# annikabrundyn/driving-dirty

Measured on AMD Instinct MI355X. Metric: 6-view scenes/sec fwd+bwd, roadmap model bs=32, higher is better.
Workload: dtype f32

## Files before the change

### driving-dirty_amd/csrc/linear.hip

```cpp
#include "dd_common.h"

namespace {

constexpr int KT = 64;
constexpr int WROW = KT + 4;
constexpr int NTD = 32;

template <int MT, bool GT>
__device__ __forceinline__ void linear_fwd_body(const float* __restrict__ X, const float* __restrict__ Wt, const float* __restrict__ bias,
                                                float* __restrict__ Y, float* __restrict__ part, int M, int N, int K, int tiles_per_split,
                                                unsigned char* __restrict__ Y8, float tau) {
  __shared__ __attribute__((aligned(16))) float wl[128 * WROW];
  __shared__ __attribute__((aligned(16))) float xl[MT * 32 * WROW];
  const int tid = threadIdx.x, lane = tid & 63;
  const int wave = __builtin_amdgcn_readfirstlane(tid >> 6);
  const int h = lane >> 5, r = lane & 31;
  const int n0 = blockIdx.x * 128;
  const int ntiles = (K + KT - 1) / KT;
  const int t0 = blockIdx.y * tiles_per_split;
  const int t1 = min(t0 + tiles_per_split, ntiles);
  const int lrow = tid >> 4, lch = tid & 15;

  f32x4 wreg[8], xreg[2 * MT];
  auto fetch = [&](int t) {
    const int kc = t * KT + lch * 4;
    const bool kok = kc < K;
#pragma unroll
    for (int p = 0; p < 8; ++p) {
      const int n = n0 + p * 16 + lrow;
      const f32x4 v = __builtin_nontemporal_load((const f32x4*)(Wt + (long)min(n, N - 1) * K + min(kc, K - 4)));
      wreg[p] = (kok && n < N) ? v : f32x4{0.f, 0.f, 0.f, 0.f};
    }
#pragma unroll
    for (int p = 0; p < 2 * MT; ++p) {
      const int m = p * 16 + lrow;
      const f32x4 v = *(const f32x4*)(X + (long)min(m, M - 1) * K + min(kc, K - 4));
      xreg[p] = (kok && m < M) ? v : f32x4{0.f, 0.f, 0.f, 0.f};
    }
  };

  f32x16 acc[MT];
#pragma unroll
  for (int mt = 0; mt < MT; ++mt)
#pragma unroll
    for (int i = 0; i < 16; ++i) acc[mt][i] = 0.f;

  if (t0 < t1) fetch(t0);
  for (int t = t0; t < t1; ++t) {
#pragma unroll
    for (int p = 0; p < 8; ++p) *(f32x4*)(wl + (p * 16 + lrow) * WROW + lch * 4) = wreg[p];
#pragma unroll
    for (int p = 0; p < 2 * MT; ++p) *(f32x4*)(xl + (p * 16 + lrow) * WROW + lch * 4) = xreg[p];
    __syncthreads();
    if (t + 1 < t1) fetch(t + 1);
#pragma unroll
    for (int s = 0; s < KT / 8; ++s) {
      const f32x4 b4 = *(const f32x4*)(wl + (wave * 32 + r) * WROW + 8 * s + 4 * h);
#pragma unroll
      for (int mt = 0; mt < MT; ++mt) {
        const f32x4 a4 = *(const f32x4*)(xl + (mt * 32 + r) * WROW + 8 * s + 4 * h);
        acc[mt] = DD_MFMA(a4.x, b4.x, acc[mt]);
        acc[mt] = DD_MFMA(a4.y, b4.y, acc[mt]);
        acc[mt] = DD_MFMA(a4.z, b4.z, acc[mt]);
        acc[mt] = DD_MFMA(a4.w, b4.w, acc[mt]);
      }
    }
    __syncthreads();
  }

  const int n = n0 + wave * 32 + r;
  const bool direct = gridDim.y == 1;
  const float bv = (direct && bias && n < N) ? bias[n] : 0.f;
  if constexpr (GT) {
    unsigned char* tile = (unsigned char*)wl;
#pragma unroll
    for (int mt = 0; mt < MT; ++mt)
#pragma unroll
      for (int i = 0; i < 16; ++i) {
        float sig, l1p;
        dd_sigmoid_softplus(acc[mt][i] + bv, sig, l1p);
        tile[(mt * 32 + dd_acc_row(i, lane)) * 128 + wave * 32 + r] = sig > tau;
      }
    __syncthreads();
    const bool vec = N % 16 == 0 && (uintptr_t)Y8 % 16 == 0;
    const int c = (tid & 7) * 16;
#pragma unroll
    for (int p = 0; p < MT; ++p) {
      const int m = p * 32 + (tid >> 3);
      if (m >= M || n0 + c >= N) continue;
      unsigned char* dst8 = Y8 + (long)m * N + n0 + c;
      if (vec) {
        *(u32x4*)dst8 = *(const u32x4*)(tile + m * 128 + c);
      } else {
        for (int j = 0; j < min(16, N - n0 - c); ++j) dst8[j] = tile[m * 128 + c + j];
      }
    }
  } else {
    float* dst = direct ? Y : part + (long)blockIdx.y * M * N;
#pragma unroll
    for (int mt = 0; mt < MT; ++mt)
#pragma unroll
      for (int i = 0; i < 16; ++i) {
        const int m = mt * 32 + dd_acc_row(i, lane);
        if (m < M && n < N) dst[(long)m * N + n] = acc[mt][i] + bv;
      }
  }
}

template <int MT>
__global__ __launch_bounds__(256) void linear_fwd_kernel(const float* __restrict__ X, const float* __restrict__ Wt,
                                                         const float* __restrict__ bias, float* __restrict__ Y,
                                                         float* __restrict__ part, int M, int N, int K,
                                                         int tiles_per_split) {
  linear_fwd_body<MT, false>(X, Wt, bias, Y, part, M, N, K, tiles_per_split, nullptr, 0.f);
}

template <int MT>
__global__ __launch_bounds__(256) void linear_sigmoid_gt_kernel(const float* __restrict__ X, const float* __restrict__ Wt,
                                                                const float* __restrict__ bias, unsigned char* __restrict__ Y8, float tau,
                                                                int M, int N, int K) {
  linear_fwd_body<MT, true>(X, Wt, bias, nullptr, nullptr, M, N, K, (K + KT - 1) / KT, Y8, tau);
}

__global__ __launch_bounds__(256) void splits_reduce_kernel(const float* __restrict__ part, const float* __restrict__ bias,
                                                            float* __restrict__ out, long elems, int nsplit, int ncols) {
  __shared__ float red[32][8];
  const int el = threadIdx.x & 7, g = threadIdx.x >> 3;
  const long e = (long)blockIdx.x * 8 + el;
  float s0 = 0.f, s1 = 0.f, s2 = 0.f, s3 = 0.f;
  if (e < elems) {
    int s = g;
    for (; s + 96 < nsplit; s += 128) {
      s0 += part[(long)(s + 0) * elems + e];
      s1 += part[(long)(s + 32) * elems + e];
      s2 += part[(long)(s + 64) * elems + e];
      s3 += part[(long)(s + 96) * elems + e];
    }
    for (; s < nsplit; s += 32) s0 += part[(long)s * elems + e];
  }
  red[g][el] = (s0 + s1) + (s2 + s3);
  __syncthreads();
  if (g != 0 || e >= elems) return;
  float v = 0.f;
#pragma unroll
  for (int i = 0; i < 32; ++i) v += red[i][el];
  if (bias) v += bias[e % ncols];
  out[e] = v;
}

__global__ __launch_bounds__(256) void splits_reduce_few_kernel(const float* __restrict__ part, const float* __restrict__ bias,
                                                                float* __restrict__ out, long elems, int nsplit, int ncols) {
  const long e = (long)blockIdx.x * blockDim.x + threadIdx.x;
  if (e >= elems) return;
  float v = 0.f;
  for (int s = 0; s < nsplit; ++s) v += part[(long)s * elems + e];
  if (bias) v += bias[e % ncols];
  out[e] = v;
}

static inline void launch_splits_reduce(const float* part, const float* bias, float* out, long elems, int nsplit, int ncols, hipStream_t st) {
  if (nsplit >= 16)
    hipLaunchKernelGGL(splits_reduce_kernel, dim3((unsigned)((elems + 7) / 8)), dim3(256), 0, st, part, bias, out, elems, nsplit, ncols);
  else
    hipLaunchKernelGGL(splits_reduce_few_kernel, dim3((unsigned)((elems + 255) / 256)), dim3(256), 0, st, part, bias, out, elems, nsplit, ncols);
}

template <int MT>
__global__ __launch_bounds__(256) void linear_dgrad_kernel(const float* __restrict__ dY, const float* __restrict__ Wt,
                                                           float* __restrict__ dX, float* __restrict__ part, int M,
                                                           int N, int K, int tiles_per_split) {
  __shared__ __attribute__((aligned(16))) float wl[NTD * 128];
  __shared__ __attribute__((aligned(16))) float gl[MT * 32 * (NTD + 4)];
  constexpr int GROW = NTD + 4;
  const int tid = threadIdx.x, lane = tid & 63;
  const int wave = __builtin_amdgcn_readfirstlane(tid >> 6);
  const int h = lane >> 5, r = lane & 31;
  const int c0 = blockIdx.x * 128;
  const int ntiles = (N + NTD - 1) / NTD;
  const int t0 = blockIdx.y * tiles_per_split;
  const int t1 = min(t0 + tiles_per_split, ntiles);
// ... 177 lines not shown
  }

#pragma unroll
  for (int a = 0; a < TN; ++a) {
#pragma unroll
    for (int i = 0; i < 16; ++i) {
      const int n = nbase + 32 * a + dd_acc_row(i, lane);
      if (n < N && kok) __builtin_nontemporal_store(f32x4{acc[a][0][i], acc[a][1][i], acc[a][2][i], acc[a][3][i]}, (f32x4*)(dW + (long)n * K + kcol));
    }
    if (db && kg == 0) {
      const float tot = bsum[a] + __shfl_xor(bsum[a], 32);
      const int n = nbase + 32 * a + r;
      if (h == 0 && n < N) db[n] = tot;
    }
  }
}

__global__ __launch_bounds__(256) void column_sum_kernel(const float* __restrict__ dY, float* __restrict__ db, int M, int N) {
  const int c = (blockIdx.x * 256 + threadIdx.x) * 4;
  if (c >= N) return;
  if (c + 4 <= N && N % 4 == 0) {
    f32x4 s = {0.f, 0.f, 0.f, 0.f};
    for (int m = 0; m < M; ++m) s += *(const f32x4*)(dY + (long)m * N + c);
    *(f32x4*)(db + c) = s;
  } else {
    for (int j = c; j < min(c + 4, N); ++j) {
      float s = 0.f;
      for (int m = 0; m < M; ++m) s += dY[(long)m * N + j];
      db[j] = s;
    }
  }
}

int pick_mt(int M) { return M <= 32 ? 1 : (M <= 64 ? 2 : 0); }
constexpr int MCHUNK = 64;

int pick_split(int blocks_other, int ntiles) {
  if (ntiles <= 8) return 1;
  int want = (2 * DD_NUM_CU + blocks_other - 1) / blocks_other;
  want = max(1, min(want, ntiles));
  return min(want, 512);
}

int check_linear(const char* who, int M, int N, int K) {
  DD_REQUIRE(M > 0 && N > 0 && K > 0, DD_ERR_BAD_ARG, "%s: non-positive size", who);
  DD_REQUIRE(K % 4 == 0 && N % 4 == 0, DD_ERR_UNSUPPORTED, "%s: N = %d and K = %d must be multiples of 4", who, N, K);
  return 0;
}

}

extern "C" {

int64_t dd_linear_workspace_bytes(int32_t m, int32_t n, int32_t k) {
  const int64_t mc = m < MCHUNK ? m : MCHUNK;
  const int64_t fwd = ((n + 127) / 128 >= 2 * DD_NUM_CU) ? 0 : (int64_t)512 * mc * n * 4;
  const int64_t dgr = ((k + 127) / 128 >= 2 * DD_NUM_CU) ? 0 : (int64_t)512 * mc * k * 4;
  return (fwd > dgr ? fwd : dgr) + 16;
}

int dd_linear_fwd(const float* x, const float* w, const float* bias, float* y, int32_t m, int32_t n, int32_t k,
                  void* workspace, int64_t workspace_bytes, void* stream) {
  if (int rc = check_linear("linear_fwd", m, n, k)) return rc;
  DD_REQUIRE(x && w && y, DD_ERR_BAD_ARG, "linear_fwd: NULL pointer");
  hipStream_t st = (hipStream_t)stream;
  const int nblk = (n + 127) / 128, ntiles = (k + KT - 1) / KT;
  const int split = pick_split(nblk, ntiles);
  const int tps = (ntiles + split - 1) / split;
  const int nsplit = (ntiles + tps - 1) / tps;
  float* part = (float*)workspace;
  if (nsplit > 1)
    DD_REQUIRE(workspace && workspace_bytes >= (int64_t)nsplit * min(m, MCHUNK) * n * 4, DD_ERR_WORKSPACE, "linear_fwd: workspace too small");
  const dim3 grid(nblk, nsplit);
  for (int m0 = 0; m0 < m; m0 += MCHUNK) {
// ... 38 lines not shown
}

int dd_linear_dgrad(const float* dy, const float* w, float* dx, int32_t m, int32_t n, int32_t k, void* workspace,
                    int64_t workspace_bytes, void* stream) {
  if (int rc = check_linear("linear_dgrad", m, n, k)) return rc;
  DD_REQUIRE(dy && w && dx, DD_ERR_BAD_ARG, "linear_dgrad: NULL pointer");
  hipStream_t st = (hipStream_t)stream;
  const int kblk = (k + 127) / 128, ntiles = (n + NTD - 1) / NTD;
  const int split = pick_split(kblk, ntiles);
  const int tps = (ntiles + split - 1) / split;
  const int nsplit = (ntiles + tps - 1) / tps;
  float* part = (float*)workspace;
  if (nsplit > 1)
    DD_REQUIRE(workspace && workspace_bytes >= (int64_t)nsplit * min(m, MCHUNK) * k * 4, DD_ERR_WORKSPACE, "linear_dgrad: workspace too small");
  const dim3 grid(kblk, nsplit);
  for (int m0 = 0; m0 < m; m0 += MCHUNK) {
    const int mc = min(MCHUNK, m - m0);
    const float* dyc = dy + (long)m0 * n;
    float* dxc = dx + (long)m0 * k;
    switch (pick_mt(mc)) {
      case 1: hipLaunchKernelGGL(linear_dgrad_kernel<1>, grid, dim3(256), 0, st, dyc, w, dxc, part, mc, n, k, tps); break;
      default: hipLaunchKernelGGL(linear_dgrad_kernel<2>, grid, dim3(256), 0, st, dyc, w, dxc, part, mc, n, k, tps); break;
    }
    DD_LAUNCH_CHECK("linear_dgrad");
    if (nsplit > 1) {
      const long elems = (long)mc * k;
      launch_splits_reduce(part, nullptr, dxc, elems, nsplit, k, st);
      DD_LAUNCH_CHECK("linear_dgrad reduce");
    }
  }
  return 0;
}

int dd_column_sum(const float* dy, float* dbias, int32_t m, int32_t n, void* stream) {
  DD_REQUIRE(dy && dbias && m > 0 && n > 0, DD_ERR_BAD_ARG, "column_sum: bad argument");
  DD_REQUIRE(n % 4 != 0 || ((uintptr_t)dy | (uintptr_t)dbias) % 16 == 0, DD_ERR_BAD_ARG, "column_sum: buffers must be 16-byte aligned");
  hipLaunchKernelGGL(column_sum_kernel, dim3((unsigned)((n + 1023) / 1024)), dim3(256), 0, (hipStream_t)stream, dy, dbias, m, n);
  DD_LAUNCH_CHECK("column_sum");
  return 0;
}

int dd_linear_wgrad(const float* dy, const float* x, float* dw, float* dbias, int32_t m, int32_t n, int32_t k,
                    void* stream) {
  DD_REQUIRE(m > 0 && n > 0 && k > 0, DD_ERR_BAD_ARG, "linear_wgrad: non-positive size");
  DD_REQUIRE(dy && x && dw, DD_ERR_BAD_ARG, "linear_wgrad: NULL pointer");
  hipStream_t st = (hipStream_t)stream;
  if (k >= 512 && k % 4 == 0 && ((uintptr_t)x % 16 == 0) && ((uintptr_t)dw % 16 == 0)) {
    const int gk = (k + 127) / 128;
    const long total = (long)((n + 31) / 32) * gk;
    hipLaunchKernelGGL((linear_wgrad_wide_kernel<1>), dim3((unsigned)((total + 3) / 4)), dim3(256), 0, st, dy, x, dw,
                       dbias, m, n, k, gk, total);
  } else if (n <= 256 || k > n) {
    const int gk = (k + 31) / 32;
    const long total = (long)((n + 127) / 128) * gk;
    hipLaunchKernelGGL((linear_wgrad_kernel<4, 1>), dim3((unsigned)((total + 3) / 4)), dim3(256), 0, st, dy, x, dw, dbias,
                       m, n, k, gk, total);
  } else {
    const int gk = (k + 63) / 64;
    const long total = (long)((n + 31) / 32) * gk;
    hipLaunchKernelGGL((linear_wgrad_kernel<1, 2>), dim3((unsigned)((total + 3) / 4)), dim3(256), 0, st, dy, x, dw, dbias,
                       m, n, k, gk, total);
  }
  DD_LAUNCH_CHECK("linear_wgrad");
  return 0;
}

// ... 2 lines not shown
```

### driving-dirty_amd/joint.py

```python
import torch
from torch import nn

from . import ops
from .autoencoder import BasicAE
from .lightning import LightningModule, hparam, pretrained_ae
from .roadmap import predict_map
from .spatial import RoadMapBoxesMergingCNN, SpatialMappingCNN, bb_coord_to_map, boxes_from_map, per_sample_inputs


class JointRoadMapBBox(LightningModule):
    def __init__(self, hparams):
        super().__init__()
        self.hparams = hparams
        self.ae = pretrained_ae(hparams)
        self.ae.decoder = None
        self.ae.encoder.c3_only = False
        self.fc1 = nn.Linear(self.ae.latent_dim, 800 * 800)
        self.space_map_cnn = SpatialMappingCNN()
        self.box_merge = RoadMapBoxesMergingCNN()
        precision = hparam(hparams, "precision", None)
        if precision is not None:
            if precision not in ("fp32", "fp32x3"):
                raise ValueError(f"precision must be 'fp32' or 'fp32x3', got {precision!r}")
            self.box_merge.precision = precision

    def forward(self, x, rm):
        x = tuple(t.contiguous() for t in x) if isinstance(x, (tuple, list)) else x.contiguous()
        wide4 = ops.wide_image(x)
        feat, pooled = self.ae.encoder.conv_feature_and_pooled(wide4)
        boxes = self.box_merge(feat, self.space_map_cnn(x), rm).squeeze(1)
        z = self.ae.encoder._tail(pooled, (None, None))
        logits = ops.linear(z, self.fc1.weight, self.fc1.bias).reshape(-1, 800, 800)
        return logits, boxes

    def predict_boxes(self, x, rm, threshold=0.5, min_pixels=1, max_boxes=256, fit="extent", pad_px=0.5, split_px=0, grow_iters=None):
        with torch.no_grad():
            return boxes_from_map(self(x, rm)[1], threshold, min_pixels, max_boxes, fit, pad_px, split_px, grow_iters)

    def predict_road_map(self, x, threshold=None):
        views = tuple(t.contiguous() for t in x) if isinstance(x, (tuple, list)) else x.contiguous()
        return predict_map(self, lambda: self.ae.encoder.forward_nhwc4(ops.wide_image(views)), threshold)

    def training_step(self, batch, batch_idx):
        sample, target, road_image = batch
        if per_sample_inputs(sample, road_image) and all(t.numel() % 4 == 0 for t in road_image) and len(road_image) <= ops.PTR_TABLE_MAX:
            dev = sample[0].device
            b = len(sample)
            target_bb = bb_coord_to_map(target, dev).to(dev).float()
            logits, boxes = self(tuple(sample), tuple(road_image))
            loss_rm, _ = ops.BceWithLogitsProbs.apply(logits.reshape(b, -1), tuple(road_image))
        else:
            sample = torch.stack(tuple(sample), dim=0) if isinstance(sample, (tuple, list)) else sample
            target_rm = torch.stack(tuple(road_image), dim=0).float()
            target_bb = bb_coord_to_map(target, sample.device).to(sample.device).float()
            logits, boxes = self(sample, target_rm.unsqueeze(1))
            b = target_rm.size(0)
            loss_rm = ops.BceWithLogits.apply(logits.reshape(b, -1), target_rm.reshape(b, -1))
        loss_bb = ops.BceProbs.apply(boxes.reshape(b, -1), target_bb.reshape(b, -1))
        loss = loss_rm + loss_bb
        return {"loss": loss, "log": {"train_loss": loss, "roadmap_loss": loss_rm, "bbox_loss": loss_bb}}

    def configure_optimizers(self):
        return torch.optim.Adam(self.parameters(), lr=self.hparams.learning_rate)
```

### driving-dirty_amd/ops.py

```python
import ctypes as C
import os

import torch

from . import _lib
from . import ddp as _ddp
from ._lib import ConvDesc, call, check, size

EPI_NONE, EPI_BIAS, EPI_BIAS_RELU, EPI_RELU_MASK = 0, 1, 2, 3
PACK_FWD, PACK_DGRAD_S1, PACK_DGRAD_S2 = 0, 1, 2

_stream, _p, _dev = _lib.stream, _lib.ptr, _lib.dev


def conv_out(n, stride):
    return (n + 2 - 3) // stride + 1


def conv_desc(batch, h, w, cin_real, stride, rows_per_task=0):
    return ConvDesc(batch, h, w, cin_real, 4 if cin_real == 3 else cin_real, 32, 3, stride, 1, rows_per_task)


def stitch6(views, mask_slot=-1, want_nhwc4=True, want_nchw=False, want_target=False):
    b, n, c, h, w = views.shape
# ... 844 lines not shown
                        g1 = conv_wino_dgrad_bits(g2, p2d, s1, d2)
                    else:
                        g1 = conv_dgrad_bits(g2, p2d, s1, d2)
                    dw1, db1 = conv_wgrad(x4, g1, d1)

            if C2_DGRAD_FIRST:
                c2_data_gradient()
                for hook in MFMA_PHASE2_HOOKS:
                    hook()
                c2_weight_gradient()
            else:
                c2_weight_gradient()
                for hook in MFMA_PHASE2_HOOKS:
                    hook()
                c2_data_gradient()
            del g2
            if reduced is not None:
                torch.cuda.current_stream().wait_event(reduced)
        return None, dw1, db1, dw2, db2, dw3, db3, None, None


def encoder_conv_stack(x4, c1, c2, c3, pool, rows_per_task=0):
    return EncoderConvStack.apply(x4, c1.weight, c1.bias, c2.weight, c2.bias, c3.weight, c3.bias, pool, rows_per_task)


def _linear_ws(m, n, k, device):
    nbytes = size("dd_linear_workspace_bytes", m, n, k)
    return torch.empty(nbytes, device=device, dtype=torch.uint8), nbytes


RANKB = {}


class Linear(torch.autograd.Function):

    @staticmethod
    def forward(ctx, x, weight, bias):
        m, k = x.shape
        n = weight.shape[0]
        _dev(x, "x")
        _dev(weight, "weight", (n, k))
        if bias is not None:
            _dev(bias, "bias", (n,))
        y = torch.empty((m, n), device=x.device, dtype=torch.float32)
        ws, nbytes = _linear_ws(m, n, k, x.device)
        call("dd_linear_fwd", x, weight, bias, y, m, n, k, ws, nbytes)
        ctx.save_for_backward(x, weight)
        ctx.has_bias = bias is not None
        return y

    @staticmethod
    def backward(ctx, dy):
        x, weight = ctx.saved_tensors
        m, k = x.shape
        n = weight.shape[0]
        dy = dy.contiguous()
        dx = dw = db = None
        if ctx.needs_input_grad[0]:
            dx = torch.empty_like(x)
            ws, nbytes = _linear_ws(m, n, k, x.device)
            call("dd_linear_dgrad", dy, weight, dx, m, n, k, ws, nbytes)
        sync = _ddp.FACTOR_SYNC.get(weight.data_ptr()) if _ddp.FACTOR_SYNC else None
        fused = RANKB.get(weight.data_ptr()) if RANKB else None
        taken = 0
        if sync is not None and ctx.needs_input_grad[1] and sync.linear_factors(weight, x, dy):
            if ctx.has_bias and ctx.needs_input_grad[2] and not (fused is not None and fused.factor_bias(weight, sync.world * m)):
                db = column_sum(dy)
        elif fused is not None and ctx.needs_input_grad[1] and (taken := fused.linear_factors(weight, x, dy)):
            if taken == 1 and ctx.has_bias and ctx.needs_input_grad[2]:
                db = column_sum(dy)
        elif ctx.needs_input_grad[1] or (ctx.has_bias and ctx.needs_input_grad[2]):
            dw = torch.empty_like(weight)
            db = torch.empty(n, device=x.device, dtype=torch.float32) if ctx.has_bias else None
            call("dd_linear_wgrad", dy, x, dw, db, m, n, k)
        return dx, dw, db


def linear(x, weight, bias):
    x = x.contiguous()
    if _ddp.FACTOR_SYNC and torch.is_grad_enabled() and weight.requires_grad:
        sync = _ddp.FACTOR_SYNC.get(weight.data_ptr())
        if sync is not None:
            sync.linear_input(weight, x)
    return Linear.apply(x, weight, bias)


def linear_sigmoid_gt(x, weight, bias, tau):
    x = x.detach().contiguous()
    m, k = x.shape
    n = weight.shape[0]
    _dev(x, "x")
    _dev(weight.detach(), "weight", (n, k))
    if bias is not None:
        _dev(bias.detach(), "bias", (n,))
    out = torch.empty((m, n), device=x.device, dtype=torch.uint8)
    call("dd_linear_sigmoid_gt", x, weight, bias, float(tau), out, m, n, k)
    return out.view(torch.bool)


def column_sum(dy):
    m, n = dy.shape
    _dev(dy, "dy")
    db = torch.empty(n, device=dy.device, dtype=torch.float32)
    call("dd_column_sum", dy, db, m, n)
    return db


# ... 168 lines not shown
        probs = torch.empty_like(logits)
        dz = torch.empty_like(logits) if ctx.needs_input_grad[0] else None
        if isinstance(target, (tuple, list)):
            b, per = len(target), _check_masks(target, n)
            if b > PTR_TABLE_MAX:
                target = _stack_masks(target, logits.shape)
        if isinstance(target, (tuple, list)):
            table = (C.c_void_p * b)(*[t.data_ptr() for t in target])
            call("dd_bce_logits_u8_ptrs", logits, table, b, per, loss, dz, probs, 1.0, _loss_ws(n, logits.device))
            ctx.save_for_backward(dz)
            ctx.mark_non_differentiable(probs)
            ctx.set_materialize_grads(False)
            return loss, probs
        if not target.is_cuda or not target.is_contiguous() or target.shape != logits.shape:
            raise _lib.HotpathError(f"bce: target must be a contiguous GPU tensor of shape {tuple(logits.shape)}")
        if target.dtype in (torch.bool, torch.uint8):
            call("dd_bce_logits_u8", logits, target, loss, dz, probs, n, 1.0, _loss_ws(n, logits.device))
        else:
            _dev(target, "target", logits.shape)
            call("dd_bce_logits", logits, target, loss, dz, probs, n, 1.0, _loss_ws(n, logits.device))
        ctx.save_for_backward(dz)
        ctx.mark_non_differentiable(probs)
        ctx.set_materialize_grads(False)
        return loss, probs

    @staticmethod
    def backward(ctx, g, _gp):
        (dz,) = ctx.saved_tensors
        if g is None:
            return None, None
        return _scaled_loss_grad(ctx, dz, g), None


class MseLoss(torch.autograd.Function):

    @staticmethod
    def forward(ctx, pred, target):
        _dev(pred, "pred")
        _dev(target, "target", pred.shape)
        n = pred.numel()
        loss = torch.empty((), device=pred.device, dtype=torch.float32)
        da = torch.empty_like(pred) if ctx.needs_input_grad[0] else None
        call("dd_mse", pred, target, loss, da, n, 1.0, _loss_ws(n, pred.device))
        ctx.save_for_backward(da)
        return loss

    @staticmethod
    def backward(ctx, g):
        (da,) = ctx.saved_tensors
        return _scaled_loss_grad(ctx, da, g), None


class BceProbs(torch.autograd.Function):

    @staticmethod
    def forward(ctx, probs, target):
        _dev(probs, "probs")
        _dev(target, "target", probs.shape)
        n = probs.numel()
        loss = torch.empty((), device=probs.device, dtype=torch.float32)
        dp = torch.empty_like(probs) if ctx.needs_input_grad[0] else None
        call("dd_bce_probs", probs, target, loss, dp, n, 1.0, _loss_ws(n, probs.device))
        ctx.save_for_backward(dp)
        return loss

    @staticmethod
# ... 150 lines not shown
```

### driving-dirty_amd/roadmap.py

```python
from argparse import ArgumentParser

import torch
from torch import nn
from torch.nn import functional as F

from . import ops
from .autoencoder import BasicAE
from .lightning import LightningModule, hparam, pretrained_ae


def predict_map(module, latent, threshold):
    if threshold is None:
        threshold = hparam(module.hparams, "rm_threshold", None)
    tau = 0.5 if threshold is None else float(threshold)
    modes = [(m, m.training) for m in module.modules()]
    module.eval()
    try:
        with torch.no_grad():
            y = ops.linear_sigmoid_gt(latent(), module.fc1.weight, module.fc1.bias, tau)
    finally:
        for m, was in modes:
            m.training = was
    return y.reshape(y.size(0), 800, 800)

# ... 22 lines not shown
        x = torch.stack(tuple(sample), dim=0) if isinstance(sample, (tuple, list)) else sample
        return ops.stitch6(x.contiguous(), want_nhwc4=False, want_nchw=True)[1]

    def _encode(self, sample, keeps=(None, None)):
        wide4 = ops.wide_image(sample, self.ae.encoder.precision)
        return self.ae.encoder.forward_nhwc4(wide4, keeps)

    def _logits(self, x, keeps=(None, None)):
        representations = self._encode(x, keeps)
        y = ops.linear(representations, self.fc1.weight, self.fc1.bias)
        return y.reshape(y.size(0), 800, 800)

    def forward(self, x, keeps=(None, None)):
        y = self._logits(x, keeps)
        return y, ops.sigmoid(y.detach())

    @property
    def rm_threshold(self):
        return hparam(self.hparams, "rm_threshold", None)

    @rm_threshold.setter
    def rm_threshold(self, value):
        self.hparams.rm_threshold = None if value is None else float(value)

    def predict_road_map(self, x, threshold=None):
        return predict_map(self, lambda: self._encode(x), threshold)

    def _run_step(self, batch, batch_idx, step_name, keeps=(None, None)):
        sample, target, road_image = batch
        logging = self.logger is not None and batch_idx % self.hparams.output_img_freq == 0
        per_sample = tuple(road_image)
        if (step_name == "train" and not logging and 0 < len(per_sample) <= ops.PTR_TABLE_MAX and
                all(t.is_cuda and t.is_contiguous() and t.dtype in (torch.bool, torch.uint8) and t.numel() % 4 == 0 for t in per_sample)):
            pred_rm = self._logits(sample, keeps)
            b = len(per_sample)
            loss, probs = ops.BceWithLogitsProbs.apply(pred_rm.reshape(b, -1), per_sample)
            return loss, None, pred_rm, probs.reshape(b, 800, 800)
        masks = torch.stack(per_sample, dim=0)
        pred_rm = self._logits(sample, keeps)
        target_rm = masks.float() if (logging or step_name != "train" or masks.dtype.is_floating_point) else masks
        batch_size = masks.size(0)
        loss_target = masks if masks.dtype in (torch.bool, torch.uint8) else target_rm
        loss, probs = ops.BceWithLogitsProbs.apply(pred_rm.reshape(batch_size, -1), loss_target.reshape(batch_size, -1).contiguous())
        pred_logit_rm = probs.reshape(batch_size, 800, 800)
        if logging:
            self._log_rm_images(self.wide_stitch_six_images(sample), target_rm, pred_logit_rm, step_name)
        return loss, target_rm, pred_rm, pred_logit_rm

    def _log_rm_images(self, x, target_rm, pred_rm, step_name, limit=1):
        exp = self.logger.experiment
        step = self.trainer.global_step if self.trainer is not None else 0
        exp.add_image(f"{step_name}_input_images", x[:limit][0], step)
        exp.add_image(f"{step_name}_target_roadmaps", target_rm[:limit], step)
        exp.add_image(f"{step_name}_pred_roadmaps", pred_rm[:limit].round(), step)

    def training_step(self, batch, batch_idx):
        if self.current_epoch >= self.hparams.unfreeze_epoch_no and self.frozen:
            self.frozen = False
            self.ae.unfreeze()
        train_loss, _, _, _ = self._run_step(batch, batch_idx, step_name="train")
        return {"loss": train_loss, "log": {"train_loss": train_loss}}

    def validation_step(self, batch, batch_idx):
        val_loss, target_rm, pred_rm, pred_logit_rm = self._run_step(batch, batch_idx, step_name="valid")
        val_ts = compute_ts_road_map(target_rm, pred_logit_rm)
        val_ts_rounded = ops.threat_score(target_rm.contiguous(), pred_logit_rm.contiguous(), round_b=True)
# ... 63 lines not shown
```

### include/dd_hotpath.h

```cpp
#ifndef DD_HOTPATH_H
#define DD_HOTPATH_H

#include <stdint.h>

#ifdef __cplusplus
extern "C" {
#endif

#define DD_ABI_VERSION 4

enum {
  DD_OK = 0,
  DD_ERR_UNSUPPORTED = 1,
  DD_ERR_BAD_ARG = 2,
  DD_ERR_LAUNCH = 3,
  DD_ERR_WORKSPACE = 4
};

enum {
  DD_EPI_NONE = 0,
  DD_EPI_BIAS = 1,
  DD_EPI_BIAS_RELU = 2,
  DD_EPI_RELU_MASK = 3
};
// ... 228 lines not shown
int dd_subsample_nhwc4_u8_ptrs(const unsigned char* const* mask_ptrs, float* dst, int32_t batch, int32_t h, int32_t w,
                               int32_t oh, int32_t ow, int32_t stride, int32_t offset, void* stream);
int dd_conv1ch_fwd(const float* taps4, const float* w, const float* bias, float* y, int32_t batch, int32_t sh, int32_t sw,
                   int32_t relu, void* stream);
int dd_conv1ch_fwd_phase3(const float* taps4, const float* w, const float* bias, float* y_phase, uint32_t* relu_bits, int32_t batch,
                          int32_t sh, int32_t sw, int32_t relu, void* stream);
int dd_conv1ch_wgrad_phase3(const float* taps4, const float* g_phase, float* dw, float* dbias, int32_t batch, int32_t sh, int32_t sw,
                            void* workspace, void* stream);
int dd_phase3_scatter(const float* src_phase, float* dst, int32_t batch, int32_t oh, int32_t ow, int32_t src_ph, int32_t src_pw, int32_t off,
                      int32_t dst_cstore, int32_t dst_coff, void* stream);
int dd_phase3_gather(const float* src, float* dst_phase, int32_t batch, int32_t oh, int32_t ow, int32_t dst_ph, int32_t dst_pw, int32_t off,
                     int32_t src_cstore, int32_t src_coff, void* stream);
int64_t dd_conv1ch_wgrad_workspace_bytes(void);
int dd_conv1ch_wgrad(const float* taps4, const float* g, float* dw, float* dbias, int32_t batch, int32_t sh, int32_t sw,
                     void* workspace, void* stream);
int dd_copy_channels(const float* src, float* dst, int64_t npix, int32_t channels, int32_t src_cstore, int32_t src_coff,
                     int32_t dst_cstore, int32_t dst_coff, void* stream);
int dd_copy_channels_window(const float* src, float* dst, int32_t batch, int32_t h, int32_t w, int32_t channels, int32_t src_mem_h,
                            int32_t src_mem_w, int32_t src_y0, int32_t src_x0, int32_t src_cstore, int32_t src_coff, int32_t dst_mem_h,
                            int32_t dst_mem_w, int32_t dst_y0, int32_t dst_x0, int32_t dst_cstore, int32_t dst_coff, void* stream);
int dd_add(const float* a, const float* b, float* out, int64_t n, void* stream);
int dd_bce_probs(const float* probs, const float* target, float* loss_out, float* dprobs, int64_t n, float grad_scale,
                 void* workspace, void* stream);

int64_t dd_linear_workspace_bytes(int32_t m, int32_t n, int32_t k);
int dd_linear_fwd(const float* x, const float* w, const float* bias, float* y, int32_t m, int32_t n, int32_t k,
                  void* workspace, int64_t workspace_bytes, void* stream);
int dd_linear_dgrad(const float* dy, const float* w, float* dx, int32_t m, int32_t n, int32_t k, void* workspace,
                    int64_t workspace_bytes, void* stream);
int dd_linear_sigmoid_gt(const float* x, const float* w, const float* bias, float tau, uint8_t* out, int32_t m, int32_t n, int32_t k,
                         void* stream);
int dd_linear_wgrad(const float* dy, const float* x, float* dw, float* dbias, int32_t m, int32_t n, int32_t k,
                    void* stream);
int dd_column_sum(const float* dy, float* dbias, int32_t m, int32_t n, void* stream);

int64_t dd_threat_score_workspace_bytes(void);
int dd_threat_score(const float* a, const float* b, float* out, int64_t n, int32_t round_b, void* workspace, void* stream);

enum { DD_TARGET_F32 = 0, DD_TARGET_U8 = 1 };
int dd_ts_hist(const float* prob, const void* target, int32_t target_dtype, int64_t n, int32_t bins, int64_t* hist, void* stream);

int64_t dd_label_components_workspace_bytes(int32_t batch, int32_t height, int32_t width);
int dd_label_components(const float* maps, float threshold, int32_t* labels, int32_t batch, int32_t height, int32_t width, void* stream);

int64_t dd_component_boxes_workspace_bytes(int32_t batch, int32_t height, int32_t width);
int dd_component_boxes(const float* maps, float threshold, int32_t min_pixels, int32_t max_boxes, float* boxes, int32_t* counts, int32_t batch,
                       int32_t height, int32_t width, void* workspace, int64_t workspace_bytes, void* stream);

int64_t dd_component_obb_workspace_bytes(int32_t batch, int32_t height, int32_t width, int32_t max_boxes);
int dd_component_obb(const float* maps, float threshold, int32_t min_pixels, int32_t max_boxes, float pad_px, float* boxes, int32_t* counts,
                     int64_t* moments, int32_t batch, int32_t height, int32_t width, void* workspace, int64_t workspace_bytes, void* stream);

int64_t dd_split_components_workspace_bytes(int32_t batch, int32_t height, int32_t width, int32_t split_px, int32_t grow_iters);
int dd_split_components(const float* maps, float threshold, int32_t split_px, int32_t grow_iters, int32_t* labels, int32_t batch, int32_t height,
                        int32_t width, void* workspace, int64_t workspace_bytes, void* stream);

int64_t dd_labelled_boxes_workspace_bytes(int32_t batch, int32_t height, int32_t width);
int dd_labelled_boxes(const int32_t* labels, int32_t min_pixels, int32_t max_boxes, float* boxes, int32_t* counts, int32_t batch, int32_t height,
                      int32_t width, void* workspace, int64_t workspace_bytes, void* stream);
int64_t dd_labelled_obb_workspace_bytes(int32_t batch, int32_t height, int32_t width, int32_t max_boxes);
int dd_labelled_obb(const int32_t* labels, int32_t min_pixels, int32_t max_boxes, float pad_px, float* boxes, int32_t* counts, int64_t* moments,
                    int32_t batch, int32_t height, int32_t width, void* workspace, int64_t workspace_bytes, void* stream);

int64_t dd_box_iou_ats_workspace_bytes(const int32_t* offsets1, const int32_t* offsets2, int32_t batch);
int dd_box_iou_ats(const void* boxes1, int32_t dtype1, const int32_t* offsets1, const void* boxes2, int32_t dtype2, const int32_t* offsets2,
                   float* iou, float* ats, int32_t batch, void* workspace, int64_t workspace_bytes, void* stream);
// ... 111 lines not shown
```

Before: 4358.

## Fuse roadmap head linear, sigmoid-BCE loss, logit gradient and dgrad in one kernel

Adds a fused training kernel for the final fc1 layer. In one pass it computes the 640k-wide logits, the BCE loss against the per-sample byte masks, dZ = (sigmoid - t)*scale, and partial input gradients dX. This avoids writing the logits to memory and reading them back in a separate BCE kernel, and replaces the separate dgrad pass over the large weight matrix. Partial loss and dX slabs are reduced in a small finish kernel. The cost is that the weight gradient is still computed in backward from the stored dZ, and the single kernel uses more LDS and registers.

```diff
diff --git a/driving-dirty_amd/csrc/linear.hip b/driving-dirty_amd/csrc/linear.hip
--- a/driving-dirty_amd/csrc/linear.hip
+++ b/driving-dirty_amd/csrc/linear.hip
@@ -5,6 +5,22 @@
 constexpr int KT = 64;
 constexpr int WROW = KT + 4;
 constexpr int NTD = 32;
+
+template <int MT>
+__device__ __forceinline__ void fwd_tile_mfma(f32x16 (&acc)[MT], const float* wrow, const float* xrow, int xtile) {
+#pragma unroll
+  for (int s = 0; s < KT / 8; ++s) {
+    const f32x4 b4 = *(const f32x4*)(wrow + 8 * s);
+#pragma unroll
+    for (int mt = 0; mt < MT; ++mt) {
+      const f32x4 a4 = *(const f32x4*)(xrow + mt * xtile + 8 * s);
+      acc[mt] = DD_MFMA(a4.x, b4.x, acc[mt]);
+      acc[mt] = DD_MFMA(a4.y, b4.y, acc[mt]);
+      acc[mt] = DD_MFMA(a4.z, b4.z, acc[mt]);
+      acc[mt] = DD_MFMA(a4.w, b4.w, acc[mt]);
+    }
+  }
+}
 
 template <int MT, bool GT>
 __device__ __forceinline__ void linear_fwd_body(const float* __restrict__ X, const float* __restrict__ Wt, const float* __restrict__ bias,
@@ -53,18 +69,7 @@
     for (int p = 0; p < 2 * MT; ++p) *(f32x4*)(xl + (p * 16 + lrow) * WROW + lch * 4) = xreg[p];
     __syncthreads();
     if (t + 1 < t1) fetch(t + 1);
-#pragma unroll
-    for (int s = 0; s < KT / 8; ++s) {
-      const f32x4 b4 = *(const f32x4*)(wl + (wave * 32 + r) * WROW + 8 * s + 4 * h);
-#pragma unroll
-      for (int mt = 0; mt < MT; ++mt) {
-        const f32x4 a4 = *(const f32x4*)(xl + (mt * 32 + r) * WROW + 8 * s + 4 * h);
-        acc[mt] = DD_MFMA(a4.x, b4.x, acc[mt]);
-        acc[mt] = DD_MFMA(a4.y, b4.y, acc[mt]);
-        acc[mt] = DD_MFMA(a4.z, b4.z, acc[mt]);
-        acc[mt] = DD_MFMA(a4.w, b4.w, acc[mt]);
-      }
-    }
+    fwd_tile_mfma<MT>(acc, wl + (wave * 32 + r) * WROW + 4 * h, xl + r * WROW + 4 * h, 32 * WROW);
     __syncthreads();
   }
 
@@ -122,11 +127,11 @@
   linear_fwd_body<MT, true>(X, Wt, bias, nullptr, nullptr, M, N, K, (K + KT - 1) / KT, Y8, tau);
 }
 
-__global__ __launch_bounds__(256) void splits_reduce_kernel(const float* __restrict__ part, const float* __restrict__ bias,
-                                                            float* __restrict__ out, long elems, int nsplit, int ncols) {
+__device__ __forceinline__ void splits_reduce_block(const float* __restrict__ part, const float* __restrict__ bias, float* __restrict__ out,
+                                                    long elems, int nsplit, int ncols, long block) {
   __shared__ float red[32][8];
   const int el = threadIdx.x & 7, g = threadIdx.x >> 3;
-  const long e = (long)blockIdx.x * 8 + el;
+  const long e = block * 8 + el;
   float s0 = 0.f, s1 = 0.f, s2 = 0.f, s3 = 0.f;
   if (e < elems) {
     int s = g;
@@ -146,6 +151,11 @@
   for (int i = 0; i < 32; ++i) v += red[i][el];
   if (bias) v += bias[e % ncols];
   out[e] = v;
+}
+
+__global__ __launch_bounds__(256) void splits_reduce_kernel(const float* __restrict__ part, const float* __restrict__ bias,
+                                                            float* __restrict__ out, long elems, int nsplit, int ncols) {
+  splits_reduce_block(part, bias, out, elems, nsplit, ncols, blockIdx.x);
 }
 
 __global__ __launch_bounds__(256) void splits_reduce_few_kernel(const float* __restrict__ part, const float* __restrict__ bias,
@@ -389,6 +399,194 @@
   }
 }
 
+constexpr int HEAD_SHARES = 512;
+
+struct HeadMasks {
+  const unsigned char* p[64];
+};
+
+template <int MT, int K>
+struct HeadTile {
+  static constexpr int WS = K + 4;
+  static constexpr int GS = 128 + 4;
+  static constexpr int MB = 128 + 4;
+  static constexpr int LDS_BYTES = (128 * WS + MT * 32 * WS + MT * 32 * GS) * 4 + MT * 32 * MB;
+};
+
+template <int MT, int K>
+__global__ __launch_bounds__(256) void linear_bce_train_kernel(const float* __restrict__ X, const float* __restrict__ Wt,
+                                                               const float* __restrict__ bias, const HeadMasks tab, float* __restrict__ dZ,
+                                                               float* __restrict__ dxpart, double* __restrict__ lpart, int M, int N,
+                                                               int nshares, int bps, float gscale) {
+  using T = HeadTile<MT, K>;
+  constexpr int WS = T::WS, GS = T::GS, MB = T::MB;
+  constexpr int TPR = K / 4, RPP = 256 / TPR, NPASS = 128 / RPP;
+  constexpr int KTILES = K / 32;
+  static_assert(K == 64 || K == 128, "linear_bce_train_kernel: K = 64 or 128");
+  extern __shared__ __attribute__((aligned(16))) float head_lds[];
+  float* wl = head_lds;
+  float* xl = wl + 128 * WS;
+  float* gl = xl + MT * 32 * WS;
+  unsigned char* ml = (unsigned char*)(gl + MT * 32 * GS);
+  const int tid = threadIdx.x, lane = tid & 63;
+  const int wave = __builtin_amdgcn_readfirstlane(tid >> 6);
+  const int h = lane >> 5, r = lane & 31;
+  const int lrow = tid / TPR, lch = tid % TPR;
+  const int trow = tid >> 5, tch = tid & 31;
+  const int nblk = (N + 127) / 128;
+  const int kt = (wave + 2 * ((blockIdx.x / DD_NUM_CU) & 1)) & 3;
+
+#pragma unroll
+  for (int p = 0; p < MT * 32 / RPP; ++p) {
+    const int m = p * RPP + lrow;
+    const f32x4 v = *(const f32x4*)(X + (long)min(m, M - 1) * K + lch * 4);
+    *(f32x4*)(xl + m * WS + lch * 4) = m < M ? v : f32x4{0.f, 0.f, 0.f, 0.f};
+  }
+  const unsigned char* mp[MT * 4];
+#pragma unroll
+  for (int p = 0; p < MT * 4; ++p) {
+    const unsigned char* even = tab.p[min(2 * wave + 8 * p, M - 1)];
+    const unsigned char* odd = tab.p[min(2 * wave + 8 * p + 1, M - 1)];
+    mp[p] = h ? odd : even;
+  }
+
+  f32x4 wreg[NPASS];
+  unsigned mreg[MT * 4];
+  float breg;
+  const float* bp = bias ? bias : X;
+  const __amdgpu_buffer_rsrc_t zrs = dd_rsrc(dZ, M * N * 4);
+  auto fetch = [&](int blk) {
+    const int n0 = blk * 128;
+    breg = bp[min(n0 + wave * 32 + r, N - 1)];
+#pragma unroll
+    for (int p = 0; p < NPASS; ++p)
+      wreg[p] = __builtin_nontemporal_load((const f32x4*)(Wt + (long)min(n0 + p * RPP + lrow, N - 1) * K + lch * 4));
+    const int nc = min(n0 + tch * 4, N - 4);
+#pragma unroll
+    for (int p = 0; p < MT * 4; ++p) mreg[p] = *(const unsigned*)(mp[p] + nc);
+  };
+
+  for (int share = blockIdx.x; share < nshares; share += gridDim.x) {
+    f32x16 dacc[MT];
+#pragma unroll
+    for (int mt = 0; mt < MT; ++mt)
+#pragma unroll
+      for (int i = 0; i < 16; ++i) dacc[mt][i] = 0.f;
+    float lsum = 0.f;
+
+    const int bend = min((share + 1) * bps, nblk);
+    int blk = share * bps;
+    if (blk < bend) fetch(blk);
+    for (; blk < bend; ++blk) {
+      const int n0 = blk * 128;
+#pragma unroll
+      for (int p = 0; p < NPASS; ++p)
+        *(f32x4*)(wl + (p * RPP + lrow) * WS + lch * 4) = n0 + p * RPP + lrow < N ? wreg[p] : f32x4{0.f, 0.f, 0.f, 0.f};
+#pragma unroll
+      for (int p = 0; p < MT * 4; ++p) *(unsigned*)(ml + (trow + 8 * p) * MB + tch * 4) = mreg[p];
+      const int n = n0 + wave * 32 + r;
+      const float bv = (bias && n < N) ? breg : 0.f;
+      __syncthreads();
+      if (blk + 1 < bend) fetch(blk + 1);
+
+      f32x16 acc[MT];
+#pragma unroll
+      for (int mt = 0; mt < MT; ++mt)
+#pragma unroll
+        for (int i = 0; i < 16; ++i) acc[mt][i] = 0.f;
+#pragma unroll
+      for (int t = 0; t < K / KT; ++t) fwd_tile_mfma<MT>(acc, wl + (wave * 32 + r) * WS + t * KT + 4 * h, xl + r * WS + t * KT + 4 * h, 32 * WS);
+
+      const int he = dd_fresh_lane() >> 5;
+#pragma unroll
+      for (int mt = 0; mt < MT; ++mt)
+#pragma unroll
+        for (int i = 0; i < 16; ++i) {
+          const int m = mt * 32 + dd_acc_row_half(i, he);
+          const float z = acc[mt][i] + bv;
+          const float t = (float)ml[m * MB + wave * 32 + r];
+          float sig, l1p;
+          dd_sigmoid_softplus(z, sig, l1p);
+          const bool ok = m < M && n < N;
+          if (ok) lsum += fmaxf(z, 0.f) - z * t + l1p;
+          gl[m * GS + wave * 32 + r] = ok ? (sig - t) * gscale : 0.f;
+        }
+      dd_barrier_lds();
+
+      const int srow = 2 * wave + (dd_fresh_lane() >> 5);
+#pragma unroll
+      for (int p = 0; p < MT * 4; ++p) {
+        const int m = srow + 8 * p, nc = n0 + tch * 4;
+        dd_bstore(zrs, m < M && nc < N ? (m * N + nc) * 4 : -1, *(const f32x4*)(gl + m * GS + tch * 4));
+      }
+      if (dxpart && kt < KTILES) {
+#pragma unroll
+        for (int s = 0; s < 128 / 8; ++s) {
+          const int nb = 8 * s + 4 * h;
+          float b[4];
+#pragma unroll
+          for (int i = 0; i < 4; ++i) b[i] = wl[(nb + i) * WS + kt * 32 + r];
+#pragma unroll
+          for (int mt = 0; mt < MT; ++mt) {
+            const f32x4 a4 = *(const f32x4*)(gl + (mt * 32 + r) * GS + nb);
+            dacc[mt] = DD_MFMA(a4.x, b[0], dacc[mt]);
+            dacc[mt] = DD_MFMA(a4.y, b[1], dacc[mt]);
+            dacc[mt] = DD_MFMA(a4.z, b[2], dacc[mt]);
+            dacc[mt] = DD_MFMA(a4.w, b[3], dacc[mt]);
+          }
+        }
+      }
+      dd_barrier_lds();
+    }
+
+    if (dxpart && kt < KTILES) {
+      float* slab = dxpart + (long)share * M * K;
+      const int hs = dd_fresh_lane() >> 5;
+#pragma unroll
+      for (int mt = 0; mt < MT; ++mt)
+#pragma unroll
+        for (int i = 0; i < 16; ++i) {
+          const int m = mt * 32 + dd_acc_row_half(i, hs);
+          if (m < M) slab[(long)m * K + kt * 32 + r] = dacc[mt][i];
+        }
+    }
+
+    double d = (double)lsum;
+#pragma unroll
+    for (int o = 32; o > 0; o >>= 1) d += __shfl_down(d, o);
+    double* lred = (double*)wl;
+    if (lane == 0) lred[wave] = d;
+    __syncthreads();
+    if (tid == 0) lpart[share] = (lred[0] + lred[1]) + (lred[2] + lred[3]);
+    __syncthreads();
+  }
+}
+
+__global__ __launch_bounds__(256) void linear_bce_finish_kernel(const float* __restrict__ dxpart, float* __restrict__ dx, long elems, int nslab,
+                                                                const double* __restrict__ lpart, double inv_n, float* __restrict__ loss) {
+  if (blockIdx.x + 1 < gridDim.x) {
+    if (nslab >= 16) {
+      splits_reduce_block(dxpart, nullptr, dx, elems, nslab, 1, blockIdx.x);
+    } else if (threadIdx.x < 8 && (long)blockIdx.x * 8 + threadIdx.x < elems) {
+      const long e = (long)blockIdx.x * 8 + threadIdx.x;
+      float v = 0.f;
+      for (int s = 0; s < nslab; ++s) v += dxpart[(long)s * elems + e];
+      dx[e] = v;
+    }
+    return;
+  }
+  __shared__ double red[256];
+  double s = 0.0;
+  for (int i = threadIdx.x; i < nslab; i += 256) s += lpart[i];
+  red[threadIdx.x] = s;
+  __syncthreads();
+  for (int o = 128; o > 0; o >>= 1) {
+    if ((int)threadIdx.x < o) red[threadIdx.x] += red[threadIdx.x + o];
+    __syncthreads();
+  }
+  if (threadIdx.x == 0) loss[0] = (float)(red[0] * inv_n);
+}
+
 int pick_mt(int M) { return M <= 32 ? 1 : (M <= 64 ? 2 : 0); }
 constexpr int MCHUNK = 64;
 
@@ -397,6 +595,14 @@
   int want = (2 * DD_NUM_CU + blocks_other - 1) / blocks_other;
   want = max(1, min(want, ntiles));
   return min(want, 512);
+}
+
+void head_shares(int N, int K, int* nshares, int* bps) {
+  const int nblk = (N + 127) / 128, ntiles = (N + NTD - 1) / NTD;
+  const int split = pick_split((K + 127) / 128, ntiles);
+  const int tps = (ntiles + split - 1) / split;
+  *bps = tps % 4 == 0 ? tps / 4 : (nblk + HEAD_SHARES - 1) / HEAD_SHARES;
+  *nshares = (nblk + *bps - 1) / *bps;
 }
 
 int check_linear(const char* who, int M, int N, int K) {
@@ -501,6 +707,57 @@
   return 0;
 }
 
+int64_t dd_linear_bce_workspace_bytes(int32_t m, int32_t n, int32_t k) {
+  (void)n;
+  const int64_t mm = m > 0 ? m : 0, kk = k > 0 ? k : 0;
+  return (int64_t)HEAD_SHARES * (8 + mm * kk * 4) + 16;
+}
+
+int dd_linear_bce_train(const float* x, const float* w, const float* bias, const unsigned char* const* mask_ptrs, int32_t batch,
+                        int64_t per_sample, int32_t k, float* loss_out, float* dz, float* dx, float grad_scale, void* workspace,
+                        int64_t workspace_bytes, void* stream) {
+  DD_REQUIRE(batch > 0 && per_sample > 0 && k > 0, DD_ERR_BAD_ARG, "linear_bce_train: non-positive size");
+  DD_REQUIRE(x && w && mask_ptrs && loss_out && dz && workspace, DD_ERR_BAD_ARG, "linear_bce_train: NULL pointer");
+  DD_REQUIRE(k == 64 || k == 128, DD_ERR_UNSUPPORTED, "linear_bce_train: K = %d (64 or 128)", k);
+  DD_REQUIRE(per_sample % 4 == 0 && per_sample <= INT32_MAX / 256, DD_ERR_UNSUPPORTED,
+             "linear_bce_train: N = %ld must be a multiple of 4 (and at most %d)", (long)per_sample, INT32_MAX / 256);
+  DD_REQUIRE(batch <= 64, DD_ERR_UNSUPPORTED, "linear_bce_train: M = %d rows (at most 64)", batch);
+  DD_REQUIRE(((uintptr_t)x | (uintptr_t)w | (uintptr_t)dz | (uintptr_t)dx | (uintptr_t)workspace) % 16 == 0, DD_ERR_BAD_ARG,
+             "linear_bce_train: buffers must be 16-byte aligned");
+  HeadMasks tab;
+  for (int i = 0; i < 64; ++i) tab.p[i] = i < batch ? mask_ptrs[i] : nullptr;
+  for (int i = 0; i < batch; ++i)
+    DD_REQUIRE(tab.p[i] && (uintptr_t)tab.p[i] % 4 == 0, DD_ERR_BAD_ARG, "linear_bce_train: sample %d: NULL or misaligned mask", i);
+  const int m = batch, n = (int)per_sample, mt = pick_mt(m);
+  const int lds = mt == 1 ? (k == 64 ? HeadTile<1, 64>::LDS_BYTES : HeadTile<1, 128>::LDS_BYTES)
+                          : (k == 64 ? HeadTile<2, 64>::LDS_BYTES : HeadTile<2, 128>::LDS_BYTES);
+  int nshares, bps;
+  head_shares(n, k, &nshares, &bps);
+  const int grid = min(nshares, dd_cu_budget_internal() * (2 * lds <= 160 * 1024 ? 2 : 1));
+  const int npart = (nshares + 1) & ~1;
+  DD_REQUIRE(workspace_bytes >= (int64_t)npart * 8 + (dx ? (int64_t)nshares * m * k * 4 : 0), DD_ERR_WORKSPACE, "linear_bce_train: workspace too small");
+  double* lpart = (double*)workspace;
+  float* dxpart = dx ? (float*)(lpart + npart) : nullptr;
+  const float gscale = grad_scale / (float)((int64_t)m * n);
+  hipStream_t st = (hipStream_t)stream;
+#define DD_HEAD_LAUNCH(MT_, K_)                                                                                                         \
+  do {                                                                                                                                  \
+    if (int rc = dd_allow_lds((const void*)linear_bce_train_kernel<MT_, K_>, lds)) return rc;                                           \
+    hipLaunchKernelGGL((linear_bce_train_kernel<MT_, K_>), dim3(grid), dim3(256), lds, st, x, w, bias, tab, dz, dxpart, lpart, m, n, nshares, bps, gscale); \
+  } while (0)
+  if (mt == 1 && k == 64) DD_HEAD_LAUNCH(1, 64);
+  else if (mt == 1) DD_HEAD_LAUNCH(1, 128);
+  else if (k == 64) DD_HEAD_LAUNCH(2, 64);
+  else DD_HEAD_LAUNCH(2, 128);
+#undef DD_HEAD_LAUNCH
+  DD_LAUNCH_CHECK("linear_bce_train");
+  const long elems = (long)m * k;
+  hipLaunchKernelGGL(linear_bce_finish_kernel, dim3((unsigned)((dx ? (elems + 7) / 8 : 0) + 1)), dim3(256), 0, st, dxpart, dx, elems, nshares, lpart,
+                     1.0 / (double)((int64_t)m * n), loss_out);
+  DD_LAUNCH_CHECK("linear_bce_finish");
+  return 0;
+}
+
 int dd_column_sum(const float* dy, float* dbias, int32_t m, int32_t n, void* stream) {
   DD_REQUIRE(dy && dbias && m > 0 && n > 0, DD_ERR_BAD_ARG, "column_sum: bad argument");
   DD_REQUIRE(n % 4 != 0 || ((uintptr_t)dy | (uintptr_t)dbias) % 16 == 0, DD_ERR_BAD_ARG, "column_sum: buffers must be 16-byte aligned");
diff --git a/driving-dirty_amd/joint.py b/driving-dirty_amd/joint.py
--- a/driving-dirty_amd/joint.py
+++ b/driving-dirty_amd/joint.py
@@ -25,13 +25,16 @@
             self.box_merge.precision = precision
 
     def forward(self, x, rm):
+        z, boxes = self._latent_and_boxes(x, rm)
+        logits = ops.linear(z, self.fc1.weight, self.fc1.bias).reshape(-1, 800, 800)
+        return logits, boxes
+
+    def _latent_and_boxes(self, x, rm):
         x = tuple(t.contiguous() for t in x) if isinstance(x, (tuple, list)) else x.contiguous()
         wide4 = ops.wide_image(x)
         feat, pooled = self.ae.encoder.conv_feature_and_pooled(wide4)
         boxes = self.box_merge(feat, self.space_map_cnn(x), rm).squeeze(1)
-        z = self.ae.encoder._tail(pooled, (None, None))
-        logits = ops.linear(z, self.fc1.weight, self.fc1.bias).reshape(-1, 800, 800)
-        return logits, boxes
+        return self.ae.encoder._tail(pooled, (None, None)), boxes
 
     def predict_boxes(self, x, rm, threshold=0.5, min_pixels=1, max_boxes=256, fit="extent", pad_px=0.5, split_px=0, grow_iters=None):
         with torch.no_grad():
@@ -47,8 +50,12 @@
             dev = sample[0].device
             b = len(sample)
             target_bb = bb_coord_to_map(target, dev).to(dev).float()
-            logits, boxes = self(tuple(sample), tuple(road_image))
-            loss_rm, _ = ops.BceWithLogitsProbs.apply(logits.reshape(b, -1), tuple(road_image))
+            if ops.FUSE_HEAD_BCE and torch.is_grad_enabled():
+                z, boxes = self._latent_and_boxes(tuple(sample), tuple(road_image))
+                loss_rm = ops.linear_bce(z, self.fc1.weight, self.fc1.bias, tuple(road_image))
+            else:
+                logits, boxes = self(tuple(sample), tuple(road_image))
+                loss_rm, _ = ops.BceWithLogitsProbs.apply(logits.reshape(b, -1), tuple(road_image))
         else:
             sample = torch.stack(tuple(sample), dim=0) if isinstance(sample, (tuple, list)) else sample
             target_rm = torch.stack(tuple(road_image), dim=0).float()
diff --git a/driving-dirty_amd/ops.py b/driving-dirty_amd/ops.py
--- a/driving-dirty_amd/ops.py
+++ b/driving-dirty_amd/ops.py
@@ -900,6 +900,27 @@
 RANKB = {}
 
 
+def _linear_param_grads(weight, x, dy, need_w, need_b, has_bias):
+    m, k = x.shape
+    n = weight.shape[0]
+    dw = db = None
+    need_b = need_b and has_bias
+    sync = _ddp.FACTOR_SYNC.get(weight.data_ptr()) if _ddp.FACTOR_SYNC else None
+    fused = RANKB.get(weight.data_ptr()) if RANKB else None
+    taken = 0
+    if sync is not None and need_w and sync.linear_factors(weight, x, dy):
+        if need_b and not (fused is not None and fused.factor_bias(weight, sync.world * m)):
+            db = column_sum(dy)
+    elif fused is not None and need_w and (taken := fused.linear_factors(weight, x, dy)):
+        if taken == 1 and need_b:
+            db = column_sum(dy)
+    elif need_w or need_b:
+        dw = torch.empty_like(weight)
+        db = torch.empty(n, device=x.device, dtype=torch.float32) if has_bias else None
+        call("dd_linear_wgrad", dy, x, dw, db, m, n, k)
+    return dw, db
+
+
 class Linear(torch.autograd.Function):
 
     @staticmethod
@@ -923,24 +944,12 @@
         m, k = x.shape
         n = weight.shape[0]
         dy = dy.contiguous()
-        dx = dw = db = None
+        dx = None
         if ctx.needs_input_grad[0]:
             dx = torch.empty_like(x)
             ws, nbytes = _linear_ws(m, n, k, x.device)
             call("dd_linear_dgrad", dy, weight, dx, m, n, k, ws, nbytes)
-        sync = _ddp.FACTOR_SYNC.get(weight.data_ptr()) if _ddp.FACTOR_SYNC else None
-        fused = RANKB.get(weight.data_ptr()) if RANKB else None
-        taken = 0
-        if sync is not None and ctx.needs_input_grad[1] and sync.linear_factors(weight, x, dy):
-            if ctx.has_bias and ctx.needs_input_grad[2] and not (fused is not None and fused.factor_bias(weight, sync.world * m)):
-                db = column_sum(dy)
-        elif fused is not None and ctx.needs_input_grad[1] and (taken := fused.linear_factors(weight, x, dy)):
-            if taken == 1 and ctx.has_bias and ctx.needs_input_grad[2]:
-                db = column_sum(dy)
-        elif ctx.needs_input_grad[1] or (ctx.has_bias and ctx.needs_input_grad[2]):
-            dw = torch.empty_like(weight)
-            db = torch.empty(n, device=x.device, dtype=torch.float32) if ctx.has_bias else None
-            call("dd_linear_wgrad", dy, x, dw, db, m, n, k)
+        dw, db = _linear_param_grads(weight, x, dy, ctx.needs_input_grad[1], ctx.needs_input_grad[2], ctx.has_bias)
         return dx, dw, db
 
 
@@ -1175,6 +1184,79 @@
         return _scaled_loss_grad(ctx, dz, g), None
 
 
+FUSE_HEAD_BCE = True
+
+
+def _is_byte_mask(t):
+    return isinstance(t, torch.Tensor) and t.is_cuda and t.is_contiguous() and t.dtype in (torch.bool, torch.uint8)
+
+
+def _mask_rows(target, m, n):
+    if isinstance(target, (tuple, list)):
+        if len(target) != m or not all(_is_byte_mask(t) and t.numel() == n for t in target):
+            return None
+        rows = [t.data_ptr() for t in target]
+    elif _is_byte_mask(target) and tuple(target.shape) == (m, n):
+        rows = [target.data_ptr() + i * n for i in range(m)]
+    else:
+        return None
+    return rows if all(p % 4 == 0 for p in rows) else None
+
+
+def linear_bce_supported(x, weight, target):
+    if not (x.dim() == 2 and x.dtype == torch.float32 and weight.dtype == torch.float32 and x.is_cuda):
+        return False
+    m, k = x.shape
+    n = weight.shape[0]
+    return k in (64, 128) and n % 4 == 0 and 0 < m <= PTR_TABLE_MAX and _mask_rows(target, m, n) is not None
+
+
+class LinearBce(torch.autograd.Function):
+
+    @staticmethod
+    def forward(ctx, x, weight, bias, target):
+        m, k = x.shape
+        n = weight.shape[0]
+        _dev(x, "x")
+        _dev(weight, "weight", (n, k))
+        if bias is not None:
+            _dev(bias, "bias", (n,))
+        rows = _mask_rows(target, m, n)
+        if rows is None:
+            raise _lib.HotpathError("linear_bce: the target must be per-sample or stacked contiguous bool / uint8 GPU masks, 4-byte aligned")
+        loss = torch.empty((), device=x.device, dtype=torch.float32)
+        dz = torch.empty((m, n), device=x.device, dtype=torch.float32)
+        dx_unit = torch.empty_like(x) if ctx.needs_input_grad[0] else None
+        nbytes = size("dd_linear_bce_workspace_bytes", m, n, k)
+        ws = torch.empty(nbytes, device=x.device, dtype=torch.uint8)
+        call("dd_linear_bce_train", x, weight, bias, (C.c_void_p * m)(*rows), m, n, k, loss, dz, dx_unit, 1.0, ws, nbytes)
+        ctx.save_for_backward(x, weight, dz, dx_unit)
+        ctx.has_bias = bias is not None
+        return loss
+
+    @staticmethod
+    def backward(ctx, g):
+        x, weight, dz, dx_unit = ctx.saved_tensors
+        dx = dx_unit * g if dx_unit is not None else None
+        dz = _scaled_loss_grad(ctx, dz, g)
+        dw, db = _linear_param_grads(weight, x, dz, ctx.needs_input_grad[1], ctx.needs_input_grad[2], ctx.has_bias)
+        return dx, dw, db, None
+
+
+def linear_bce(x, weight, bias, target):
+    x = x.contiguous()
+    if not (FUSE_HEAD_BCE and linear_bce_supported(x, weight, target)):
+        logits = linear(x, weight, bias)
+        if isinstance(target, torch.Tensor):
+            target = target.reshape(logits.shape).contiguous()
+        return BceWithLogitsProbs.apply(logits, target)[0]
+    if _ddp.FACTOR_SYNC and torch.is_grad_enabled() and weight.requires_grad:
+        sync = _ddp.FACTOR_SYNC.get(weight.data_ptr())
+        if sync is not None:
+            sync.linear_input(weight, x)
+    return LinearBce.apply(x, weight, bias, target)
+
+
 class MseLoss(torch.autograd.Function):
 
     @staticmethod
diff --git a/driving-dirty_amd/roadmap.py b/driving-dirty_amd/roadmap.py
--- a/driving-dirty_amd/roadmap.py
+++ b/driving-dirty_amd/roadmap.py
@@ -78,6 +78,8 @@
         per_sample = tuple(road_image)
         if (step_name == "train" and not logging and 0 < len(per_sample) <= ops.PTR_TABLE_MAX and
                 all(t.is_cuda and t.is_contiguous() and t.dtype in (torch.bool, torch.uint8) and t.numel() % 4 == 0 for t in per_sample)):
+            if ops.FUSE_HEAD_BCE and torch.is_grad_enabled():
+                return ops.linear_bce(self._encode(sample, keeps), self.fc1.weight, self.fc1.bias, per_sample), None, None, None
             pred_rm = self._logits(sample, keeps)
             b = len(per_sample)
             loss, probs = ops.BceWithLogitsProbs.apply(pred_rm.reshape(b, -1), per_sample)
diff --git a/include/dd_hotpath.h b/include/dd_hotpath.h
--- a/include/dd_hotpath.h
+++ b/include/dd_hotpath.h
@@ -284,6 +284,10 @@
                          void* stream);
 int dd_linear_wgrad(const float* dy, const float* x, float* dw, float* dbias, int32_t m, int32_t n, int32_t k,
                     void* stream);
+int64_t dd_linear_bce_workspace_bytes(int32_t m, int32_t n, int32_t k);
+int dd_linear_bce_train(const float* x, const float* w, const float* bias, const unsigned char* const* mask_ptrs, int32_t batch,
+                        int64_t per_sample, int32_t k, float* loss_out, float* dz, float* dx, float grad_scale, void* workspace,
+                        int64_t workspace_bytes, void* stream);
 int dd_column_sum(const float* dy, float* dbias, int32_t m, int32_t n, void* stream);
 
 int64_t dd_threat_score_workspace_bytes(void);
```

New measurement: 4384 (median of 6 runs). About the same (+0.6%).
